# Baran-phys/IEA-GAN

Hardware: AMD Instinct MI355X
Metric: events/sec (40x250x768) per G+D train step (higher is better)
Workload: dtype bf16; 1 GPU; BASELINE configs[1]: 1 event (40x1x256x768) per GPU per step, hinge loss only, RRM on, DiffAugment on, ortho reg + Adam + EMA in the timed region, fp32 master weights, 4 synthetic events in rotation; parallelism=dp1, hip_graph=True

## Files before the change

iea-gan_amd/_hip.py:

```python
from __future__ import annotations

import ctypes as C
import os

import torch

_HERE = os.path.dirname(os.path.abspath(__file__))
LIB_PATH = os.path.join(_HERE, "libieagan_hip.so")
CONV_FP8_NOSCALE = 8
CONV_FP8 = 4
CONV_NO_LDS_WEIGHTS = 2
CONV_FORCE_GATHER = 1
B1_OCC2, B1_OCC3, B1_TP32 = 1, 2, 4
BWD_NO_REDUCE = 16
PXD_BINS = 251
PXD_CLUSTER_COLUMNS = {"size_spectrum": (0, 64), "charge_spectrum": (64, 256), "seed_spectrum": (320, 256), "size_u_spectrum": (576, 32),
                       "size_v_spectrum": (608, 32)}
PXD_CLUSTER_BINS = 640
PROLOGUE_BWD_SLOTS = 64
AUG_SLOTS = 128
BNB_REPL = 8
STAT_REPL = 32
SN_FIELDS = 16

vp, fp, lp, ip = C.c_void_p, C.c_void_p, C.c_void_p, C.c_void_p


class SrcDesc(C.Structure):
    _fields_ = [("x", vp), ("Cx", C.c_int), ("Hs", C.c_int), ("Ws", C.c_int), ("rs", C.c_int),
                ("scale", vp), ("shift", vp), ("aff_nstride", C.c_int), ("relu", C.c_int)]


class ConvDesc(C.Structure):
    _fields_ = [("N", C.c_int), ("H", C.c_int), ("W", C.c_int), ("Cin", C.c_int), ("Cout", C.c_int),
                ("taps", C.c_int), ("Kpad", C.c_int), ("src", SrcDesc), ("w", vp), ("bias", vp),
                ("ra", vp), ("Cra", C.c_int), ("Ca", C.c_int), ("ra_rs", C.c_int), ("ra_scale", C.c_float), ("rb", vp),
                ("Crb", C.c_int), ("mask", vp), ("out", vp), ("stats", vp), ("n_per_event", C.c_int), ("flags", C.c_int),
                ("bnb_scale", vp), ("bnb_shift", vp), ("bnb_nstride", C.c_int), ("bnb_relu", C.c_int), ("stats_slots", C.c_int)]


class WgradDesc(C.Structure):
# ... 21 lines not shown

class DStemDesc(C.Structure):
    _fields_ = [("img", vp), ("N", C.c_int), ("H", C.c_int), ("W", C.c_int), ("w_in", vp), ("b_in", vp), ("w1", vp), ("b1", vp), ("wsc", vp),
                ("bsc", vp), ("h1", vp), ("p0", vp), ("sc", vp), ("dh1", vp), ("dp0", vp), ("w1_bwd", vp), ("dw_in", vp), ("db_in", vp),
                ("dw1", vp), ("db1", vp)]


class ProfRec(C.Structure):
    _fields_ = [("name", C.c_char * 96), ("launches", C.c_long), ("ms", C.c_double),
                ("flops", C.c_double), ("bytes", C.c_double), ("bytes_min", C.c_double)]


ABI_VERSION = 12
i, f, l = C.c_int, C.c_float, C.c_long
_SIGS = {
    "ieagan_abi_version": [],
    "ieagan_prof_enable": [i],
    "ieagan_prof_reset": [],
    "ieagan_prof_collect": [C.POINTER(ProfRec), i],
    "ieagan_conv_forward": [C.POINTER(ConvDesc), vp],
    "ieagan_conv_wgrad": [C.POINTER(WgradDesc), i, vp],
    "ieagan_conv_wgrad_workspace": [C.POINTER(WgradDesc), i],
    "ieagan_conv1x1_bwd": [C.POINTER(Conv1x1BwdDesc), vp],
    "ieagan_conv1x1_bwd_workspace": [C.POINTER(Conv1x1BwdDesc)],
    "ieagan_conv1x1_bwd_supported": [i, i, i, i],
    "ieagan_conv3x3_bwd": [C.POINTER(Conv3x3BwdDesc), vp],
    "ieagan_conv3x3_bwd_workspace": [C.POINTER(Conv3x3BwdDesc)],
    "ieagan_conv3x3_bwd_supported": [i, i, i, i, i, i, i],
    "ieagan_conv3x3_bwd_slots": [C.POINTER(Conv3x3BwdDesc)],
    "ieagan_conv1x1_bwd_slots": [C.POINTER(Conv1x1BwdDesc)],
    "ieagan_wgrad_reduce": [vp, vp, i, i, i, i, vp],
    "ieagan_wgrad_reduce_batched": [C.POINTER(ReduceItem), i, vp],
    "ieagan_conv_stats_slots": [C.POINTER(ConvDesc)],
    "ieagan_d_stem_fwd": [C.POINTER(DStemDesc), vp],
    "ieagan_d_stem_bwd": [C.POINTER(DStemDesc), vp],
    "ieagan_effgrad": [vp, vp, vp, vp, vp, l, i, i, vp],
    "ieagan_prologue_bwd": [vp, vp, i, vp, vp, i, i, i, vp, vp, vp, i, i, i, i, vp, i, i, i, i, vp],
    "ieagan_bn_finalize_fwd": [vp, f, vp, vp, i, i, f, f, i, vp, vp, vp, vp, vp, i, i, i, i, vp, vp],
    "ieagan_bn_finalize_bwd": [vp, vp, vp, i, i, vp, f, i, vp, vp, i, vp, i, i, i, i, vp, vp],
    "ieagan_bn_finalize_fwd_scratch": [i, i, i],
    "ieagan_bn_finalize_bwd_scratch": [i, i, i, i],
    "ieagan_res_bwd": [vp, i, vp, i, i, i, i, i, i, vp],
    "ieagan_nchw_to_nhwc": [vp, vp, vp, i, i, i, i, vp],
    "ieagan_nhwc_to_nchw": [vp, vp, i, i, i, vp],
    "ieagan_channel_stats": [vp, vp, l, i, vp],
    "ieagan_conv_1toC": [vp, vp, vp, vp, vp, i, i, i, i, i, vp],
    "ieagan_conv_1toC_bnb": [vp, vp, vp, vp, vp, vp, i, i, vp, vp, vp, i, i, i, i, i, i, vp],
    "ieagan_conv_1toC_bnb_slots": [i, i, i, i],
    "ieagan_conv_Cto1": [vp, vp, vp, i, i, vp, vp, vp, i, i, i, i, i, i, vp],
    "ieagan_wgrad_c1": [vp, vp, vp, vp, vp, i, i, vp, i, i, i, i, i, vp],
    "ieagan_sn_backward_batched": [vp, vp, i, vp, vp, vp, vp, vp],
    "ieagan_sn_forward": [vp, vp, i, vp, i, vp, vp, vp, vp, f, i, vp],
    "ieagan_sn_backward": [vp, vp, i, i, i, i, i, i, vp, vp, vp, i, vp, vp, i, vp],
    "ieagan_sn_backward_stack": [vp, vp, vp, vp, i, vp, vp, vp, vp, i, vp],
    "ieagan_nl_attention_fwd": [vp, vp, vp, vp, vp, i, i, i, i, i, vp],
    "ieagan_nl_attention_bwd": [vp, vp, vp, vp, vp, vp, vp, vp, vp, vp, i, i, i, i, i, vp],
    "ieagan_rrm_attention_fwd": [vp, vp, vp, i, i, i, i, vp],
    "ieagan_rrm_attention_bwd": [vp, vp, vp, vp, i, i, i, i, vp],
    "ieagan_slin_fwd": [vp, vp, vp, vp, vp, vp, vp, vp, vp, i, i, i, i, f, vp],
    "ieagan_slin_bwd": [vp, vp, vp, vp, vp, vp, vp, vp, vp, vp, i, i, i, i, vp],
    "ieagan_ln_fwd": [vp, vp, vp, vp, vp, vp, i, i, f, i, vp],
    "ieagan_ln_bwd": [vp, vp, vp, vp, vp, vp, vp, vp, vp, i, i, vp],
    "ieagan_embed_norm_fwd": [vp, vp, vp, vp, i, i, vp],
    "ieagan_embed_norm_bwd": [vp, vp, vp, vp, vp, i, i, vp],
    "ieagan_loss_block": [vp, vp, vp, vp, vp, C.POINTER(C.c_float), f, vp, vp, vp, vp, vp, i, i, vp],
    "ieagan_loss_block_events": [vp, vp, vp, vp, vp, C.POINTER(C.c_float), f, vp, vp, vp, vp, vp, i, i, i, vp],
# ... 82 lines not shown
```

iea-gan_amd/csrc/api.hip:

```cpp
#include <stdarg.h>
#include <stdio.h>
#include <string.h>

#include <map>
#include <mutex>
#include <string>
#include <vector>

#include "common.h"
#include "conv_args.h"

static thread_local char g_err[512] = "";

void ieagan_set_error(const char* fmt, ...) {
    va_list ap;
    va_start(ap, fmt);
    vsnprintf(g_err, sizeof(g_err), fmt, ap);
    va_end(ap);
}

extern "C" const char* ieagan_last_error(void) { return g_err; }
extern "C" int ieagan_abi_version(void) { return IEAGAN_ABI_VERSION; }

struct ProfEvt {
// ... 66 lines not shown
            strncpy(r.name, e.name.c_str(), sizeof(r.name) - 1);
        }
        r.launches += 1;
        r.ms += ms;
        r.flops += e.flops;
        r.bytes += e.bytes;
        r.bytes_min += e.bytes_min;
    }
    prof_clear_locked();
    int n = 0;
    for (auto& kv : agg) {
        if (n >= cap) break;
        out[n++] = kv.second;
    }
    return n;
}

extern "C" int ieagan_conv_forward(const ieagan_conv_desc* d, void* stream) {
    CHECK_ARG(d != nullptr && d->src.x != nullptr && d->w != nullptr && d->out != nullptr, "conv_forward: null pointer");
    return conv_gather_launch(*d, (hipStream_t)stream);
}

extern "C" int ieagan_conv_stats_slots(const ieagan_conv_desc* d) {
    CHECK_ARG(d != nullptr, "conv_stats_slots: null pointer");
    g_plan.on = true;
    g_plan.slots = -1;
    const int rc = conv_gather_launch(*d, nullptr);
    g_plan.on = false;
    if (rc < 0) return rc;
    CHECK_ARG(g_plan.slots > 0, "conv_stats_slots: the dispatch reached no launch site");
    return g_plan.slots;
}

extern "C" int ieagan_conv_wgrad(const ieagan_wgrad_desc* d, int use_tr_read, void* stream) {
    CHECK_ARG(d != nullptr && d->src.x != nullptr && d->g != nullptr && d->dw != nullptr, "conv_wgrad: null pointer");
    return conv_wgrad_launch(*d, (hipStream_t)stream, use_tr_read);
}

__global__ void selftest_tr_kernel(const bf16* __restrict__ in, bf16* __restrict__ out) {
    __shared__ __attribute__((aligned(16))) bf16 lds[64 * 16];
    const int l = threadIdx.x;
    for (int i = l; i < 64 * 16; i += 64) lds[i] = in[i];
    __syncthreads();
    const int lr = l & 15, lg = l >> 4;
    const int q = lr >> 2, p = lr & 3;
    const bf16* p0 = lds + (8 * lg + q) * 16 + 4 * p;
    const bf16* p1 = p0 + 4 * 16;
    const bf16x4 lo = __builtin_amdgcn_ds_read_tr16_b64_v4bf16((bf16x4 __attribute__((address_space(3)))*)p0);
    const bf16x4 hi = __builtin_amdgcn_ds_read_tr16_b64_v4bf16((bf16x4 __attribute__((address_space(3)))*)p1);
#pragma unroll
    for (int j = 0; j < 4; ++j) {
        out[l * 8 + j] = lo[j];
        out[l * 8 + 4 + j] = hi[j];
    }
}

extern "C" int ieagan_selftest_tr_read(const void* in, void* out, void* stream) {
    hipLaunchKernelGGL(selftest_tr_kernel, dim3(1), dim3(64), 0, (hipStream_t)stream, (const bf16*)in, (bf16*)out);
    CHECK_LAUNCH("selftest_tr_read");
    return 0;
}
```

iea-gan_amd/csrc/conv1x1_tile.hip:

```cpp
#include "common.h"
#include "conv_args.h"
#include "conv_common.h"

namespace {

template <int KC>
__device__ __forceinline__ int tkey(int r) { return KC == 128 ? (r & 15) : KC == 64 ? ((r >> 1) & 7) : ((r >> 2) & 3); }
template <int KC>
__device__ __forceinline__ int toff(int r, int c) { return r * KC + ((c ^ tkey<KC>(r)) << 3); }

template <bool AFF, bool RELU>
__device__ __forceinline__ void pro8(float (&v)[8], const bf16x8& raw, const SrcDesc& s, int n, int c, const float* aff) {
#pragma unroll
    for (int i = 0; i < 8; ++i) v[i] = bf2f(raw[i]);
    xform8<AFF, RELU>(v, s, n, c, aff);
}

}

template <bool AFF, bool RELU, int RS, int NT, int KC, bool BNB>
__global__ __launch_bounds__(256, 3) void conv1x1_tile_kernel(ConvArgs a) {
    constexpr int CPR = KC / 8;
    constexpr int EROWS = 16;
    constexpr int ABYTES = 128 * KC * 2, BBYTES = NT * 16 * KC * 2;
    constexpr int EPIB = 4 * EROWS * EpiLds<NT>::LDW * 4;
    constexpr int ASZ = ABYTES > EPIB ? ABYTES : EPIB;
    static_assert(EPIB >= 4 * STATS_SX_FLOATS * 4, "epilogue buffer doubles as the statistics scratch");
    __shared__ __attribute__((aligned(16))) char smem[ASZ + BBYTES];
    __shared__ float red[4 * NT * 16 * 2];
    __shared__ __attribute__((aligned(32))) float aff_s[AFF ? 2 * AFF_MAXC : 8];
    bf16* atile = (bf16*)smem;
    bf16* btile = (bf16*)(smem + ASZ);
    float* epi = (float*)smem;
    const int lane = threadIdx.x & 63, wave = threadIdx.x >> 6;
    const int lr = lane & 15, lg = lane >> 4;
    const int H = a.H, W = a.W, HW = H * W;
    const long M = (long)a.N * HW;
    const int gy = a.Cout / (NT * 16);
    int vid = blockIdx.x;
    {
        const int tot = gridDim.x, q = tot / 8, r = tot % 8, xcd = vid % 8;
        vid = (xcd < r ? xcd * (q + 1) : r * (q + 1) + (xcd - r) * q) + vid / 8;
    }
    const int bx = vid / gy;
    const long m_blk = (long)bx * 128;
    const long m_base = m_blk + wave * 32;
    const int n_base = (vid % gy) * NT * 16;
    const int n_img = (int)(m_blk / HW);
    if (AFF) stage_aff(aff_s, a.src, n_img, a.Cin);
    const float* affp = AFF ? aff_s : nullptr;
    const bf16* xsrc = (const bf16*)a.src.x;

    f32x4 acc[2][NT];
#pragma unroll
// ... 80 lines not shown
                    for (int q = 0; q < 4; ++q) {
                        float v[8];
                        pro8<AFF, RELU>(v, raw[jj][q], a.src, n, min(ch, a.Cin - 8), affp);
#pragma unroll
                        for (int i = 0; i < 8; ++i) s8[i] += v[i];
                    }
                    bf16x8 o;
#pragma unroll
                    for (int i = 0; i < 8; ++i) o[i] = f2bf(0.25f * s8[i]);
                    if (m_blk + p >= M || ch >= a.Cin) o = zero8();
                    *(bf16x8*)(atile + toff<KC>(p, c)) = o;
                }
            }
        }
        __syncthreads();
#pragma unroll
        for (int ks = 0; ks < KC / 32; ++ks) {
            bf16x8 af[2], bf[NT];
#pragma unroll
            for (int mt = 0; mt < 2; ++mt) af[mt] = *(const bf16x8*)(atile + toff<KC>(wave * 32 + mt * 16 + lr, ks * 4 + lg));
#pragma unroll
            for (int nt = 0; nt < NT; ++nt) bf[nt] = *(const bf16x8*)(btile + toff<KC>(nt * 16 + lr, ks * 4 + lg));
#pragma unroll
            for (int mt = 0; mt < 2; ++mt)
#pragma unroll
                for (int nt = 0; nt < NT; ++nt) acc[mt][nt] = __builtin_amdgcn_mfma_f32_16x16x32_bf16(af[mt], bf[nt], acc[mt][nt], 0, 0, 0);
        }
    }
    __syncthreads();

    float s1[8], s2[8];
#pragma unroll
    for (int i = 0; i < 8; ++i) s1[i] = s2[i] = 0.f;
    const bool need_hw = (a.ra != nullptr && a.ra_rs != 0) || (BNB && a.bnb_scale != nullptr);
    auto pix = [&](int row, long& m, int& n, int& h, int& w) -> bool {
        m = m_base + row;
        n = h = w = 0;
        if (m >= M) return false;
        if (need_hw) {
            n = (int)(m / HW);
            const int rem = (int)(m - (long)n * HW);
            h = rem / W;
            w = rem - h * W;
        }
        return true;
    };
#pragma unroll
    for (int half = 0; half < 2; ++half) {
        auto pixh = [&](int row, long& m, int& n, int& h, int& w) -> bool { return pix(row + 16 * half, m, n, h, w); };
        const f32x4(&sub)[1][NT] = *reinterpret_cast<const f32x4(*)[1][NT]>(&acc[half]);
        conv_epilogue<BNB, NT, 1, (RS != 2)>(a, sub, epi + wave * EROWS * EpiLds<NT>::LDW, n_base, pixh, s1, s2);
    }
    if (a.stats != nullptr) {
        __syncthreads();
        const int event = (a.n_per_event > 0) ? (int)(m_blk / ((long)a.n_per_event * HW)) : 0;
        stats_flush<NT>(a, s1, s2, n_base, red, epi, bx, event);
    }
}

template <bool AFF, bool RELU, int RS, bool BNB>
static int tile_dispatch(const ConvArgs& a, hipStream_t st) {
    const long M = (long)a.N * a.H * a.W;
    const unsigned gx = (unsigned)((M + 127) / 128);
    const int n_events_t = (a.stats != nullptr && a.n_per_event > 0) ? a.N / a.n_per_event : 1;
#define TL(NTV, KCV)                                                                                                                    \
    {                                                                                                                                   \
        CONV_PLAN_POINT((int)(gx / n_events_t), 1)                                                                                      \
        hipLaunchKernelGGL((conv1x1_tile_kernel<AFF, RELU, RS, NTV, KCV, BNB>), dim3(gx * (a.Cout / (NTV * 16))), dim3(256), 0, st, a);     \
        return 1;                                                                                                                       \
    }
#define BY_KC(NTV)                      \
    if (a.Cin <= 32) TL(NTV, 32)        \
    else if (a.Cin == 64) TL(NTV, 64)   \
    else TL(NTV, 128)
    if (a.Cout % 64 == 0) { BY_KC(4) }
    else { BY_KC(2) }
#undef BY_KC
#undef TL
    return 0;
}

int conv1x1_tile_launch(const ConvArgs& a, hipStream_t st) {
    if (a.taps != 1 || (a.src.rs != 0 && a.src.rs != 2) || a.Cout % 32 != 0 || a.Cin % 8 != 0) return 0;
    if (!(a.Cin <= 32 || a.Cin == 64 || a.Cin % 128 == 0) || a.Kpad != ((a.Cin + 31) / 32) * 32) return 0;
    const long HW = (long)a.H * a.W, M = (long)a.N * HW;
    if (M < (a.src.rs == 2 ? 1024 : 4096)) return 0;
    if (M < 16384 && a.Cin > 256) return 0;
    const bool aff = a.src.scale != nullptr, relu = a.src.relu != 0;
    if (aff && (HW % 128 != 0 || a.Cin > AFF_MAXC)) return 0;
    if (a.bnb_scale != nullptr) {
        if (aff || relu || a.src.rs != 0) return 0;
        return tile_dispatch<false, false, 0, true>(a, st);
    }
    if (a.src.rs == 0) {
        if (aff && relu) return tile_dispatch<true, true, 0, false>(a, st);
        if (aff) return tile_dispatch<true, false, 0, false>(a, st);
        if (relu) return tile_dispatch<false, true, 0, false>(a, st);
        return tile_dispatch<false, false, 0, false>(a, st);
    }
    if (aff && relu) return tile_dispatch<true, true, 2, false>(a, st);
    if (aff) return tile_dispatch<true, false, 2, false>(a, st);
    if (relu) return tile_dispatch<false, true, 2, false>(a, st);
    return tile_dispatch<false, false, 2, false>(a, st);
}
```

iea-gan_amd/csrc/conv_common.h:

```cpp
#pragma once
#include "common.h"
#include "conv_args.h"

#define AFF_MAXC 512
__device__ __forceinline__ void stage_aff(float* aff, const SrcDesc& s, int n, int Cin) {
    for (int i = threadIdx.x; i < Cin; i += 256) {
        aff[i] = s.scale[(long)n * s.aff_nstride + i];
        aff[AFF_MAXC + i] = s.shift[(long)n * s.aff_nstride + i];
    }
}

template <bool AFF, bool RELU>
__device__ __forceinline__ void xform8(float (&v)[8], const SrcDesc& s, int n, int c, const float* aff = nullptr) {
    if (AFF) {
        f32x8 sc, sh;
        if (aff != nullptr) {
            typedef const __attribute__((address_space(3))) f32x8* lds_f32x8;
            sc = *(lds_f32x8)(aff + c);
            sh = *(lds_f32x8)(aff + AFF_MAXC + c);
        } else {
            sc = *(const f32x8*)(s.scale + (long)n * s.aff_nstride + c);
            sh = *(const f32x8*)(s.shift + (long)n * s.aff_nstride + c);
        }
#pragma unroll
// ... 169 lines not shown
                int n, h, w;
                long mm;
                pix(row, mm, n, h, w);
                const bf16* p = (const bf16*)a.ra + (((long)n * (2 * H) + 2 * h) * (2 * W) + 2 * w) * a.Cra + co0;
                const long rs_ = (long)2 * W * a.Cra;
                const bf16x8 t0 = *(const bf16x8*)p, t1 = *(const bf16x8*)(p + a.Cra), t2 = *(const bf16x8*)(p + rs_),
                             t3 = *(const bf16x8*)(p + rs_ + a.Cra);
#pragma unroll
                for (int i = 0; i < 8; ++i) rv[i] = 0.25f * (bf2f(t0[i]) + bf2f(t1[i]) + bf2f(t2[i]) + bf2f(t3[i]));
            }
#pragma unroll
            for (int i = 0; i < 8; ++i) v[i] += a.ra_scale * rv[i];
        } else if (rb_here) {
            const bf16x8 t = EARLY ? rs_r[it] : *(const bf16x8*)((const bf16*)a.rb + m * a.Crb + (co0 - a.Ca));
#pragma unroll
            for (int i = 0; i < 8; ++i) v[i] += bf2f(t[i]);
        }
        bf16x8 o;
#pragma unroll
        for (int i = 0; i < 8; ++i) {
            o[i] = f2bf(v[i]);
            if (!bnb) {
                s1[i] += v[i];
                s2[i] += v[i] * v[i];
            }
        }
        *(bf16x8*)((bf16*)a.out + m * a.Cout + co0) = o;
    }
    __builtin_amdgcn_fence(__ATOMIC_SEQ_CST, "wavefront");
    __builtin_amdgcn_wave_barrier();
}


template <bool AFF, bool RELU, int RS>
__device__ __forceinline__ bf16x8 gather8(const SrcDesc& s, int H, int W, int n, int hh, int ww, int c, bool ok,
                                          const float* aff = nullptr) {
    ok = ok && (hh >= 0) && (hh < H) && (ww >= 0) && (ww < W);
    if (!ok) return zero8();
    if (RS == 2) {
        float acc[8];
#pragma unroll
        for (int i = 0; i < 8; ++i) acc[i] = 0.f;
#pragma unroll
        for (int q = 0; q < 4; ++q) {
            const bf16x8 raw = *(const bf16x8*)((const bf16*)s.x + (((long)n * s.Hs + 2 * hh + (q >> 1)) * s.Ws + 2 * ww + (q & 1)) * s.Cx + c);
            float v[8];
#pragma unroll
            for (int i = 0; i < 8; ++i) v[i] = bf2f(raw[i]);
            xform8<AFF, RELU>(v, s, n, c, aff);
#pragma unroll
            for (int i = 0; i < 8; ++i) acc[i] += v[i];
        }
        bf16x8 o;
#pragma unroll
        for (int i = 0; i < 8; ++i) o[i] = f2bf(0.25f * acc[i]);
        return o;
    }
    const int sh_ = (RS == 1) ? (hh >> 1) : hh, sw_ = (RS == 1) ? (ww >> 1) : ww;
    const bf16x8 raw = *(const bf16x8*)((const bf16*)s.x + (((long)n * s.Hs + sh_) * s.Ws + sw_) * s.Cx + c);
    if (!AFF && !RELU) return raw;
    if (!AFF && RELU) return relu8(raw);
    float v[8];
#pragma unroll
    for (int i = 0; i < 8; ++i) v[i] = bf2f(raw[i]);
    xform8<AFF, RELU>(v, s, n, c, aff);
    bf16x8 o;
// ... 6 lines not shown
```

iea-gan_amd/csrc/conv_igemm.hip:

```cpp
#include "common.h"
#include "conv_args.h"
#include "conv_common.h"
#include <stdio.h>

template <int TAPS, bool AFF, bool RELU, int RS, int NT, bool LAFF, bool BNB = false>
__global__ __launch_bounds__(256, 4) void conv_gather_kernel(ConvArgs a) {
    constexpr int EROWS = (NT >= 2) ? 16 : 32;
    __shared__ __attribute__((aligned(16))) float epi[4 * EROWS * EpiLds<NT>::LDW];
    __shared__ float red[4 * NT * 16 * 2];
    __shared__ __attribute__((aligned(32))) float aff_s[LAFF ? 2 * AFF_MAXC : 8];
    const int lane = threadIdx.x & 63, wave = threadIdx.x >> 6;
    const int lr = lane & 15, lg = lane >> 4;
    const int H = a.H, W = a.W, HW = H * W;
    const long M = (long)a.N * HW;
    const bool sk = NT == 1 && (a.flags & CONV_INTERNAL_SPLITK) != 0;
    const int ppb = sk ? 32 : 128;
    const long m_base = sk ? (long)blockIdx.x * 32 : ((long)blockIdx.x * 4 + wave) * 32;
    const int n_base = blockIdx.y * NT * 16;

    int pn[2], ph[2], pw[2];
    bool pv[2];
#pragma unroll
    for (int mt = 0; mt < 2; ++mt) {
        const long m = m_base + mt * 16 + lr;
// ... 428 lines not shown
    const bool small = ntiles * ((a.Cout + 63) / 64) < 512;
    const bool kp_ok = a.Kpad == ((9 * a.Cin + 31) / 32) * 32;
    if (!kp_ok) {
        if (a.Cout % 64 == 0 && !small) HALO_LAUNCH(4, 0, 0)
        else if (a.Cout % 32 == 0 && !(small && ntiles * (a.Cout / 32) < 512)) HALO_LAUNCH(2, 0, 0)
        else HALO_LAUNCH(1, 0, 0)
    }
    else if (a.Cin == 16 && a.Cout == 16) HALO_LAUNCH(1, 3, 16)
    else if (a.Cin == 32 && a.Cout == 32) HALO_LAUNCH(2, 6, 32)
    else if (a.Cin == 64 && a.Cout == 64 && ntiles >= 1024) HALO_LAUNCH(4, 11, 64)
    else if (a.Cin == 64 && a.Cout % 64 == 0 && !small) HALO_LAUNCH(4, 0, 64)
    else if (a.Cin == 128 && a.Cout % 64 == 0 && !small) HALO_LAUNCH(4, 0, 128)
    else if (a.Cin == 128 && a.Cout % 32 == 0 && !(small && ntiles * (a.Cout / 32) < 512)) HALO_LAUNCH(2, 0, 128)
    else if (a.Cin == 64 && a.Cout % 32 == 0 && !(small && ntiles * (a.Cout / 32) < 512)) HALO_LAUNCH(2, 0, 64)
    else if (a.Cout % 64 == 0 && !small) HALO_LAUNCH(4, 0, 0)
    else if (a.Cout % 32 == 0 && !(small && ntiles * (a.Cout / 32) < 512)) HALO_LAUNCH(2, 0, 0)
    else HALO_LAUNCH(1, 0, 0)
#undef HALO_LAUNCH
    return 0;
}

template <int RS>
static int launch_halo_pro(const ConvArgs& a, hipStream_t st) {
    const bool aff = a.src.scale != nullptr, relu = a.src.relu != 0;
    if (aff && relu) return launch_halo_nt<true, true, RS>(a, st);
    if (aff) return launch_halo_nt<true, false, RS>(a, st);
    if (relu) return launch_halo_nt<false, true, RS>(a, st);
    if (RS == 0 && a.bnb_scale != nullptr) return launch_halo_nt<false, false, (RS == 0 ? 0 : RS), (RS == 0)>(a, st);
    return launch_halo_nt<false, false, RS>(a, st);
}

int conv_gather_launch(const ConvArgs& a, hipStream_t st) {
    CHECK_ARG(a.taps == 1 || a.taps == 9, "conv: taps must be 1 or 9 (got %d)", a.taps);
    CHECK_ARG((a.flags & ~(IEAGAN_CONV_FORCE_GATHER | IEAGAN_CONV_NO_LDS_WEIGHTS | IEAGAN_CONV_FP8 | IEAGAN_CONV_FP8_NOSCALE)) == 0, "conv: unknown flag bits 0x%x", a.flags);
    CHECK_ARG(a.Cin % 8 == 0 && a.Cout % 8 == 0, "conv: Cin/Cout must be multiples of 8 (%d,%d)", a.Cin, a.Cout);
    CHECK_ARG(a.Kpad % 32 == 0 && a.Kpad >= a.taps * a.Cin, "conv: bad Kpad %d", a.Kpad);
    CHECK_ARG(a.src.rs >= 0 && a.src.rs <= 2, "conv: bad resample mode %d", a.src.rs);
    CHECK_ARG(a.src.Cx % 8 == 0, "conv: source channel stride must be a multiple of 8");
    CHECK_ARG((a.src.scale == nullptr) == (a.src.shift == nullptr), "conv: scale/shift must come together");
    if (a.src.rs == 1) CHECK_ARG(a.H == 2 * a.src.Hs && a.W == 2 * a.src.Ws, "conv: upsample geometry mismatch");
    if (a.src.rs == 2) CHECK_ARG(2 * a.H == a.src.Hs && 2 * a.W == a.src.Ws, "conv: pool geometry mismatch");
    if (a.src.rs == 0) CHECK_ARG(a.H == a.src.Hs && a.W == a.src.Ws, "conv: geometry mismatch");
    if (a.ra) CHECK_ARG(a.Ca <= a.Cout && a.Ca <= a.Cra && a.Ca % 8 == 0 && a.Cra % 8 == 0, "conv: residual channel slice out of range");
    if (a.ra && a.ra_rs == 1) CHECK_ARG(a.H % 2 == 0 && a.W % 2 == 0, "conv: upsampled residual needs even H, W");
    if (a.rb) CHECK_ARG(a.Crb % 8 == 0 && a.Crb >= a.Cout - a.Ca, "conv: bad residual-B channel count");
    CHECK_ARG(a.n_per_event >= 0 && (a.n_per_event == 0 || a.N % a.n_per_event == 0), "conv: N=%d is not a whole number of events of %d images", a.N, a.n_per_event);
    if (a.bnb_scale != nullptr)
        CHECK_ARG(a.src.scale == nullptr && a.src.relu == 0 && a.src.rs == 0 && a.bnb_shift != nullptr && a.mask != nullptr && a.stats != nullptr && a.n_per_event == 1 && a.bias == nullptr && a.Cout % 8 == 0 &&
                  (a.bnb_nstride == 0 || a.bnb_nstride >= a.Cout), "conv: BatchNorm-backward epilogue needs a plain prologue, shift, x (mask), per-image accumulators (n_per_event = 1), no bias");
    if (a.stats != nullptr && a.n_per_event > 0 && a.n_per_event < a.N)
        CHECK_ARG(((long)a.n_per_event * a.H * a.W) % 128 == 0, "conv: per-event statistics need n_per_event*H*W %% 128 == 0 (%d*%d*%d)", a.n_per_event, a.H, a.W);
    const double flops = 2.0 * a.N * a.H * a.W * (double)a.Cout * a.taps * a.Cin;
    double bytes = 2.0 * a.N * ((double)a.src.Hs * a.src.Ws * a.Cin + (double)a.H * a.W * a.Cout);
    const double bytes_min = bytes;
    if (a.mask) bytes += 2.0 * a.N * (double)a.H * a.W * a.Cout;
    if (a.ra) bytes += 2.0 * a.N * (double)a.H * a.W * a.Ca * (a.ra_rs == 1 ? 0.25 : (a.ra_rs == 2 ? 4.0 : 1.0));
    if (a.rb) bytes += 2.0 * a.N * (double)a.H * a.W * (a.Cout - a.Ca);
    const bool halo = a.taps == 9 && a.src.rs != 2 && a.W >= 16 && a.H >= 4 && a.Cin % 16 == 0 && !(a.flags & IEAGAN_CONV_FORCE_GATHER) &&
                      (size_t)(HT_H + 2) * (HT_W + 2) * (a.Cin * 2 + 16) <= 150 * 1024 && a.Cin <= AFF_MAXC;
    char tag[64] = "";
    if (prof_tags_on())
        snprintf(tag, sizeof(tag), "ci%d co%d %dx%d rs%d a%d r%d res%d%s", a.Cin, a.Cout, a.H, a.W, a.src.rs, a.src.scale != nullptr,
                 a.src.relu, a.ra ? a.ra_rs + 1 : 0, a.mask ? " mask" : "");
    ProfScope prof(a.taps == 9 ? (halo ? "conv3x3_halo" : "conv3x3_gather") : "conv1x1_gather", flops, bytes, st, tag, bytes_min);
    int rc;
    if (halo) {
        rc = (a.flags & IEAGAN_CONV_NO_LDS_WEIGHTS) ? 0 : conv3x3_lds_launch(a, st);
        if (rc < 0) return rc;
        if (rc == 0 && !(a.flags & IEAGAN_CONV_NO_LDS_WEIGHTS)) rc = conv3x3_ws_launch(a, st);
        if (rc < 0) return rc;
        if (rc == 0) rc = (a.src.rs == 0) ? launch_halo_pro<0>(a, st) : launch_halo_pro<1>(a, st);
        else rc = 0;
    } else if (a.taps == 9) {
        if (a.src.rs == 0) rc = launch_gather_pro<9, 0>(a, st);
        else if (a.src.rs == 1) rc = launch_gather_pro<9, 1>(a, st);
        else { ieagan_set_error("conv: 3x3 with pooled source is not instantiated"); return IEAGAN_EINVAL; }
    } else {
        if (a.src.rs == 0) {
            if (!(a.flags & IEAGAN_CONV_FORCE_GATHER) && conv1x1_stream_launch(a, st)) rc = 0;
            else if (!(a.flags & IEAGAN_CONV_FORCE_GATHER) && conv1x1_tile_launch(a, st)) rc = 0;
            else rc = launch_gather_pro<1, 0>(a, st);
        }
        else if (a.src.rs == 2) {
            if (!(a.flags & IEAGAN_CONV_FORCE_GATHER) && conv1x1_tile_launch(a, st)) rc = 0;
            else rc = launch_gather_pro<1, 2>(a, st);
        }
        else { ieagan_set_error("conv: 1x1 with upsampled source is not instantiated"); return IEAGAN_EINVAL; }
    }
    if (conv_plan_ctx().on) return rc;
    CHECK_LAUNCH("conv_forward");
    return rc;
}
```

iea-gan_amd/ops.py:

```python
from __future__ import annotations

import math
import types
from typing import Optional

import torch

import _hip as H
from _hip import STAT_REPL

BF16 = torch.bfloat16


def _kpad(k: int) -> int:
    return (k + 31) // 32 * 32


class _ZeroPool:
    CHUNK = 8 << 20

    def __init__(self):
        self.buf, self.pos = {}, {}

    def take(self, n: int, device) -> torch.Tensor:
# ... 16 lines not shown


def reset_zero_pool():
    _ZEROS.reset()


def zeros(shape, device) -> torch.Tensor:
    n = 1
    for d in (shape if isinstance(shape, (tuple, list, torch.Size)) else (shape,)):
        n *= int(d)
    return _ZEROS.take(n, device).view(shape)


def new_stats(C: int, device, events: int = 1, slots: int = STAT_REPL) -> torch.Tensor:
    return zeros((events, slots, 2, C), device)


DIRECT_GRADS = False


class direct_grads:
    def __enter__(self):
        global DIRECT_GRADS
        self.prev, DIRECT_GRADS = DIRECT_GRADS, True

    def __exit__(self, *a):
        global DIRECT_GRADS
        DIRECT_GRADS = self.prev


class ExecOptions:
    FIELDS = dict(wgrad_side_stream=True, two_stage_wgrad=True, fuse_bn_backward=True, fuse_shortcut_grad=True,
                  fuse_1x1_backward=True, fuse_1x1_min_pixels=1 << 16, fuse_3x3_backward=True, fuse_3x3_min_pixels=1 << 16,
                  fuse_d_stem=True)
    __slots__ = tuple(FIELDS)

    def __init__(self, like=None, **kw):
        src = like if like is not None else globals().get("DEFAULTS")
        for k, v in self.FIELDS.items():
            setattr(self, k, getattr(src, k) if src is not None else v)
        self.update(**kw)

    def update(self, **kw):
        for k, v in kw.items():
            if k not in self.FIELDS:
                raise KeyError(f"unknown execution option {k!r} (have: {sorted(self.FIELDS)})")
            setattr(self, k, v)
        return self

    def as_dict(self):
        return {k: getattr(self, k) for k in self.FIELDS}


DEFAULTS = ExecOptions()


def opts_of(rec) -> "ExecOptions":
    ps = getattr(rec, "pass_", None)
    return ps.bank.opts if ps is not None else DEFAULTS


def opts_of_net(net) -> "ExecOptions":
    return (net if isinstance(net, SNBank) else net._prepare()["bank"]).opts


def set_options(net, **kw) -> "ExecOptions":
    bank = net if isinstance(net, SNBank) else net._prepare()["bank"]
# ... 390 lines not shown
        rows = 1 if events == 1 else n_images
        shape = (C,) if rows == 1 else (rows, C)
        scale = torch.empty(shape, dtype=torch.float32, device=dev)
        shift = torch.empty(shape, dtype=torch.float32, device=dev)
        mr = torch.empty(events, 2, C, dtype=torch.float32, device=dev)
        repl = int(stats.shape[1]) if stats is not None else 0
        H.call("ieagan_bn_finalize_fwd", H.ptr(stats), float(count), gain.data_ptr(), bias.data_ptr(), 0, 0, float(eps),
               float(momentum), int(training), run_mean.data_ptr(), run_var.data_ptr(), scale.data_ptr(),
               shift.data_ptr(), mr.data_ptr(), rows, C, events, repl,
               H.ptr(_fin_scratch("fwd", C, events, repl, device=dev) if training else None), H.stream())
        ctx.count, ctx.training, ctx.has_stats, ctx.events, ctx.rows, ctx.repl = count, training, stats is not None, events, rows, repl
        ctx.save_for_backward(gain, mr)
        return scale, shift

    @staticmethod
    def backward(ctx, dscale, dshift):
        gain, mr = ctx.saved_tensors
        C = gain.numel()
        dev = gain.device
        E, rows = ctx.events, ctx.rows
        dgain, dbias = torch.empty_like(gain), torch.empty_like(gain)
        dstat = torch.empty(E, 2, C, dtype=torch.float32, device=dev)
        shape = (C,) if rows == 1 else (rows, C)
        dscale = dscale.contiguous() if dscale is not None else torch.zeros(shape, device=dev)
        dshift = dshift.contiguous() if dshift is not None else torch.zeros(shape, device=dev)
        H.call("ieagan_bn_finalize_bwd", dscale.data_ptr(), dshift.data_ptr(), gain.data_ptr(), 0, 0, mr.data_ptr(),
               float(ctx.count), int(ctx.training), dgain.data_ptr(), dbias.data_ptr(), 0, dstat.data_ptr(), rows, C, E, 0,
               None, H.stream())
        dstats = dstat.unsqueeze(1).expand(E, ctx.repl, 2, C) if (ctx.has_stats and ctx.training) else None
        return dstats, dgain, dbias, None, None, None, None, None, None, None, None


def _conv_launch(x, Cx, Hs, Ws, rs, scale, shift, nstride, relu, N, Hc, Wc, Cin, Cout, taps, kpad, w, bias,
                 ra, Cra, Ca, ra_rs, rb, Crb, mask, out, stats, ra_scale=1.0, npe=0, flags=0, bnb=None):
    bs, bt, bn, br = (H.ptr(bnb[0]), H.ptr(bnb[1]), int(bnb[2]), int(bool(bnb[3]))) if bnb is not None else (None, None, 0, 0)
    alloc = stats is True
    d = H.ConvDesc(N, Hc, Wc, Cin, Cout, taps, kpad, H.src_desc(x, Cx, Hs, Ws, rs, scale, shift, nstride, relu),
                   H.ptr(w), H.ptr(bias), H.ptr(ra), Cra, Ca, ra_rs, float(ra_scale), H.ptr(rb), Crb, H.ptr(mask),
                   H.ptr(out), 16 if alloc else H.ptr(stats), int(npe), int(flags), bs, bt, bn, br,
                   0 if (alloc or stats is None) else int(stats.shape[1]))
    if alloc:
        slots = H.lib().ieagan_conv_stats_slots(d)
        if slots <= 0:
            raise RuntimeError(f"ieagan_conv_stats_slots failed ({slots}): {H.lib().ieagan_last_error().decode()}")
        stats = zeros((N // npe if npe else 1, slots, 2, Cout), out.device)
        d.stats, d.stats_slots = stats.data_ptr(), slots
    H.call("ieagan_conv_forward", d, H.stream())
    return stats


_WGRAD_STREAMS = {}


def wgrad_stream(device) -> "torch.cuda.Stream":
    key = (torch.device(device).index or 0, torch.cuda.current_stream(device).cuda_stream)
    if key not in _WGRAD_STREAMS:
        _WGRAD_STREAMS[key] = torch.cuda.Stream(device=device)
    return _WGRAD_STREAMS[key]


def release_device_caches():
    _ZEROS.reset()
    _WGRAD_STREAMS.clear()
    _PLACEHOLDERS.clear()


class BNLink:
    __slots__ = ("acc",)

    def __init__(self):
        self.acc = None

class ResLink:
# ... 81 lines not shown
            b.res_out.deposit(gl, gl.stride()[2] if not gl.is_contiguous() else b.Cout, b.Ca, b.ra_rs)
        elif b.ra_rs == 0:
            if b.Ca == b.Cout and rshape[-1] == b.Cout:
                d_ra = gl
            else:
                d_ra = torch.zeros(rshape, dtype=BF16, device=b.dev)
                d_ra[..., :b.Ca] = gl[..., :b.Ca]
        else:
            d_ra = torch.empty(rshape, dtype=BF16, device=b.dev)
            H.call("ieagan_res_bwd", gl.contiguous().data_ptr(), b.Cout, d_ra.data_ptr(), rshape[-1], b.Ca, b.ra_rs, b.N, rshape[1], rshape[2],
                   H.stream())
    if b.has_rb and b.need[6]:
        d_rb = gl[..., b.Ca:]
    return d_ra, d_rb


def _fused_buffers(d, kernel, N, Cin, has_aff, dev):
    acc = ws = None
    if has_aff:
        d.bn_slots = getattr(H.lib(), f"ieagan_{kernel}_slots")(d)
        if d.bn_slots <= 0:
            raise RuntimeError(f"ieagan_{kernel}_slots failed: {H.lib().ieagan_last_error().decode()}")
        acc = zeros((N, d.bn_slots, 2, Cin), dev)
        d.bn_acc = acc.data_ptr()
    ws_n = getattr(H.lib(), f"ieagan_{kernel}_workspace")(d)
    if ws_n < 0:
        raise RuntimeError(f"ieagan_{kernel}_workspace failed: {H.lib().ieagan_last_error().decode()}")
    if ws_n > 0:
        ws = torch.empty(ws_n, dtype=torch.float32, device=dev)
        d.partials = ws.data_ptr()
    return acc, ws


def _dgrad(b, g, Cg, out, *, link=None, link_rs=0, link_scale=1.0, mask=None, stats=None, bnb=None, flags=0, npe=0):
    lg, lC, lCa = link if link is not None else (None, 0, 0)
    return _conv_launch(g, Cg, b.Hc, b.Wc, 0, None, None, 0, False, b.N, b.Hc, b.Wc, b.Cout, b.Cin, b.taps, b.rec.kpad2, b.rec.w_bwd, None,
                        lg, lC, lCa, link_rs, None, 0, mask, out, stats, ra_scale=link_scale, npe=npe, flags=flags, bnb=bnb)


def _conv_grads(dx=None, dW=None, dbias=None, dscale=None, dshift=None, d_ra=None, d_rb=None):
    return (dx, dW, dbias, dscale, dshift, d_ra, d_rb) + (None,) * 11


def _fused_bwd_launch(name, d, rec, ws, dwp, Cout, K):
    pass_ = getattr(rec, "pass_", None)
    batched = ws is not None and getattr(rec, "deferred", False) and pass_ is not None and pass_.arena is not None
    if batched:
        d.flags |= H.BWD_NO_REDUCE
    H.call(name, d, H.stream())
    if batched:
        pass_.reduces.append((ws, dwp, ws.numel() // (Cout * rec.kpad), Cout, rec.kpad, K))


def _fused_1x1_eligible(b, dout, dstats):
    rec, o, rs, relu, has_aff, res_out, res_in, need = b.rec, b.opts, b.rs, b.relu, b.has_aff, b.res_out, b.res_in, b.need
    if not o.fuse_1x1_backward:
        return False
    if b.taps != 1 or rs not in (0, 2) or not need[0] or not need[1] or b.Wc % 32 != 0 or b.N * b.Hc * b.Wc < o.fuse_1x1_min_pixels:
        return False
    if not H.lib().ieagan_conv1x1_bwd_supported(rec.cin, rec.out, rs, int(has_aff)):
        return False
    if isinstance(res_in, SumLink) or (has_aff and (rs != 0 or b.events > 1 and b.nstride == 0)):
        return False
    if res_in is not None and res_in.ready:
        if rs == 2 and not (res_out is None and not relu and not has_aff):
            return False
        if rs == 0 and res_in.mode not in (0, 1, 2):
            return False
    elif rs == 2 and res_out is None and not relu and res_in is not None:
        return False
# ... 82 lines not shown
    if dstats is not None:
        geff = torch.empty_like(g)
        if b.has_bias:
            colsum = sn_scratch(rec, "b", (STAT_REPL, Cout), dev) if (need[1] and need[2]) else zeros((STAT_REPL, Cout), dev)
        H.call("ieagan_effgrad", g.data_ptr(), b.out.data_ptr(), dstats[:, 0].contiguous().data_ptr(), geff.data_ptr(),
               H.ptr(colsum), P, Cout, b.events, H.stream())
        g = geff
    elif b.has_bias and need[2]:
        colsum = sn_scratch(rec, "b", (STAT_REPL, Cout), dev) if need[1] else zeros((STAT_REPL, Cout), dev)
        if need[1]:
            colsum_in_wgrad = True
        else:
            H.call("ieagan_effgrad", g.data_ptr(), None, None, None, colsum.data_ptr(), P, Cout, 1, H.stream())
    return g, Cg, colsum, colsum_in_wgrad


def _prologue_bwd(b, da, link, rmode):
    if rmode == 2:
        raise RuntimeError("pooled shortcut gradient cannot be added by prologue_bwd")
    dx = torch.empty(b.N, b.Hs, b.Ws, b.Cin, dtype=BF16, device=b.dev)
    acc = zeros((b.N, H.PROLOGUE_BWD_SLOTS, 2, b.Cin), b.dev) if b.has_aff else None
    H.call("ieagan_prologue_bwd", da.data_ptr(), b.x.data_ptr(), b.Cx, H.ptr(b.scale), H.ptr(b.shift), b.nstride, int(b.relu),
           b.rs, dx.data_ptr(), H.ptr(acc), None, b.N, b.Hs, b.Ws, b.Cin, H.ptr(link[0]), link[1], link[2], rmode,
           H.PROLOGUE_BWD_SLOTS if b.has_aff else 0, H.stream())
    return (dx,) + (_bn_param_grads(b.scale, acc, b.nstride) if b.has_aff else (None, None))


def _data_gradient(b, g, Cg):
    x, scale, rs, relu, has_aff, res_in = b.x, b.scale, b.rs, b.relu, b.has_aff, b.res_in
    N, Hs, Ws, Cin, dev = b.N, b.Hs, b.Ws, b.Cin, b.dev
    dx = dscale = dshift = None
    if not (b.need[0] or (has_aff and (b.need[3] or b.need[4]))):
        return dx, dscale, dshift
    da = torch.empty(N, b.Hc, b.Wc, Cin, dtype=BF16, device=dev)
    fuse_mask = relu and not has_aff and rs == 0
    plain = not relu and not has_aff
    lg = lC = lCa = lmode = None
    fan_in = res_in if isinstance(res_in, SumLink) else None
    if res_in is not None and not res_in.ready:
        res_in = None
    if res_in is not None:
        lg, lC, lCa, lmode = res_in.take()
    link = (lg, lC or 0, lCa or 0)
    bn_link = getattr(scale, "_bn_link", None) if has_aff else None
    if (b.opts.fuse_bn_backward and has_aff and rs == 0 and bn_link is not None and (Hs * Ws) % 128 == 0 and Cin % 8 == 0
            and (res_in is None or lmode in (0, 1))):
        dx = torch.empty(N, Hs, Ws, Cin, dtype=BF16, device=dev)
        up = res_in is not None and lmode == 1
        acc = _dgrad(b, g, Cg, dx, link=link, link_rs=2 if up else 0, link_scale=4.0 if up else 1.0, mask=x, stats=True,
                     bnb=(scale, b.shift, b.nstride, relu), flags=b.flags, npe=1)
        dscale, dshift = _bn_param_grads(scale, acc, b.nstride)
    elif res_in is not None and (fuse_mask or (plain and rs == 0)):
        _dgrad(b, g, Cg, da, link=link, link_rs=1 if lmode == 2 else 0, link_scale=0.25 if lmode == 2 else 1.0,
               mask=x if fuse_mask else None, flags=b.flags)
        dx = da
    elif res_in is not None and plain and rs == 2 and b.res_out is None:
        _dgrad(b, g, Cg, da, link=link)
        res_in.deposit(da, Cin, Cin, 2)
    else:
        _dgrad(b, g, Cg, da, mask=x if fuse_mask else None, flags=b.flags)
        if (fuse_mask or (plain and rs == 0)) and res_in is None:
            dx = da
        else:
            dx, dscale, dshift = _prologue_bwd(b, da, link, lmode if res_in is not None else 0)
    if fan_in is not None:
        if not (plain and rs == 0 and dx is da):
# ... 645 lines not shown
```

include/ieagan_hip.h:

```cpp
#ifndef IEAGAN_HIP_H
#define IEAGAN_HIP_H
#include <stddef.h>
#ifdef __cplusplus
extern "C" {
#endif

const char* ieagan_last_error(void);
#define IEAGAN_ABI_VERSION 12
int ieagan_abi_version(void);

int ieagan_prof_enable(int on);
int ieagan_prof_reset(void);
typedef struct { char name[96]; long launches; double ms; double flops; double bytes; double bytes_min; } ieagan_prof_rec;
int ieagan_prof_collect(ieagan_prof_rec* out, int cap);

typedef struct {
    const void* x;
    int Cx, Hs, Ws;
    int rs;
    const float* scale;
    const float* shift;
    int aff_nstride;
    int relu;
} ieagan_src_desc;

typedef struct {
    int N, H, W;
    int Cin, Cout, taps;
    int Kpad;
    ieagan_src_desc src;
    const void* w;
    const float* bias;
    const void* ra;
    int Cra, Ca, ra_rs;
    float ra_scale;
    const void* rb;
    int Crb;
    const void* mask;
    void* out;
    float* stats;
    int n_per_event;
    int flags;
    const float* bnb_scale;
    const float* bnb_shift;
    int bnb_nstride;
    int bnb_relu;
    int stats_slots;
} ieagan_conv_desc;
#define IEAGAN_CONV_FORCE_GATHER 1
#define IEAGAN_CONV_FP8 4
#define IEAGAN_CONV_FP8_NOSCALE 8
#define IEAGAN_CONV_NO_LDS_WEIGHTS 2
int ieagan_conv_forward(const ieagan_conv_desc* d, void* stream);
int ieagan_conv_stats_slots(const ieagan_conv_desc* d);

typedef struct {
    int N, H, W;
    int Cin, Cout, taps, Kpad;
    ieagan_src_desc src;
    const void* g;
    int Cg;
    float* dw;
    int tiles_per_block;
    int pad_rows;
    float* partials;
    float* colsum;
} ieagan_wgrad_desc;
int ieagan_conv_wgrad(const ieagan_wgrad_desc* d, int use_tr_read, void* stream);
long ieagan_conv_wgrad_workspace(const ieagan_wgrad_desc* d, int use_tr_read);

typedef struct {
    int N, H, W;
    int Cin, Cout, Kpad, Kpad2;
    ieagan_src_desc src;
    const void* g;
    int Cg;
    const void* y;
    const float* dstat;
    int n_per_event;
    void* geff_out;
    const void* w_bwd;
    const void* lg;
    int lC, lCa, lmode;
    void* dx;
    int out_mode;
    float* bn_acc;
// ... 183 lines not shown
```

Baseline: 30.56 events/s.

## Fuse avg-pool backward and ReLU mask into 1x1 dgrad tile epilogue

Adds a pooled-source dgrad path for 1x1 convs whose input was ReLU'd and 2x2 average-pooled. The tile kernel's epilogue now scatters the quarter-scaled gradient to the four full-resolution pixels, masked by the sign of x. This replaces writing an intermediate pooled-resolution gradient and then running a separate prologue-backward pass. A plan-mode query checks shape support first and falls back to the old path otherwise. The cost is an extra kernel instantiation and scattered 4x stores from the epilogue, and the gradient is rounded to bf16 before the 0.25 scale.

```diff
diff --git a/iea-gan_amd/_hip.py b/iea-gan_amd/_hip.py
--- a/iea-gan_amd/_hip.py
+++ b/iea-gan_amd/_hip.py
@@ -7,6 +7,7 @@
 
 _HERE = os.path.dirname(os.path.abspath(__file__))
 LIB_PATH = os.path.join(_HERE, "libieagan_hip.so")
+CONV_POOL_BWD = 16
 CONV_FP8_NOSCALE = 8
 CONV_FP8 = 4
 CONV_NO_LDS_WEIGHTS = 2
@@ -94,6 +95,7 @@
     "ieagan_wgrad_reduce": [vp, vp, i, i, i, i, vp],
     "ieagan_wgrad_reduce_batched": [C.POINTER(ReduceItem), i, vp],
     "ieagan_conv_stats_slots": [C.POINTER(ConvDesc)],
+    "ieagan_conv_pool_bwd_supported": [C.POINTER(ConvDesc)],
     "ieagan_d_stem_fwd": [C.POINTER(DStemDesc), vp],
     "ieagan_d_stem_bwd": [C.POINTER(DStemDesc), vp],
     "ieagan_effgrad": [vp, vp, vp, vp, vp, l, i, i, vp],
diff --git a/iea-gan_amd/csrc/api.hip b/iea-gan_amd/csrc/api.hip
--- a/iea-gan_amd/csrc/api.hip
+++ b/iea-gan_amd/csrc/api.hip
@@ -122,6 +122,15 @@
     return g_plan.slots;
 }
 
+extern "C" int ieagan_conv_pool_bwd_supported(const ieagan_conv_desc* d) {
+    CHECK_ARG(d != nullptr, "conv_pool_bwd_supported: null pointer");
+    g_plan.on = true;
+    g_plan.slots = -1;
+    const int rc = conv_gather_launch(*d, nullptr);
+    g_plan.on = false;
+    return rc == 0 ? 1 : 0;
+}
+
 extern "C" int ieagan_conv_wgrad(const ieagan_wgrad_desc* d, int use_tr_read, void* stream) {
     CHECK_ARG(d != nullptr && d->src.x != nullptr && d->g != nullptr && d->dw != nullptr, "conv_wgrad: null pointer");
     return conv_wgrad_launch(*d, (hipStream_t)stream, use_tr_read);
diff --git a/iea-gan_amd/csrc/conv1x1_tile.hip b/iea-gan_amd/csrc/conv1x1_tile.hip
--- a/iea-gan_amd/csrc/conv1x1_tile.hip
+++ b/iea-gan_amd/csrc/conv1x1_tile.hip
@@ -18,8 +18,8 @@
 
 }
 
-template <bool AFF, bool RELU, int RS, int NT, int KC, bool BNB>
-__global__ __launch_bounds__(256, 3) void conv1x1_tile_kernel(ConvArgs a) {
+template <bool AFF, bool RELU, int RS, int NT, int KC, bool BNB, bool PBWD>
+__device__ __forceinline__ void conv1x1_tile_body(const ConvArgs a) {
     constexpr int CPR = KC / 8;
     constexpr int EROWS = 16;
     constexpr int ABYTES = 128 * KC * 2, BBYTES = NT * 16 * KC * 2;
@@ -166,7 +166,7 @@
     float s1[8], s2[8];
 #pragma unroll
     for (int i = 0; i < 8; ++i) s1[i] = s2[i] = 0.f;
-    const bool need_hw = (a.ra != nullptr && a.ra_rs != 0) || (BNB && a.bnb_scale != nullptr);
+    const bool need_hw = PBWD || (a.ra != nullptr && a.ra_rs != 0) || (BNB && a.bnb_scale != nullptr);
     auto pix = [&](int row, long& m, int& n, int& h, int& w) -> bool {
         m = m_base + row;
         n = h = w = 0;
@@ -183,13 +183,24 @@
     for (int half = 0; half < 2; ++half) {
         auto pixh = [&](int row, long& m, int& n, int& h, int& w) -> bool { return pix(row + 16 * half, m, n, h, w); };
         const f32x4(&sub)[1][NT] = *reinterpret_cast<const f32x4(*)[1][NT]>(&acc[half]);
-        conv_epilogue<BNB, NT, 1, (RS != 2)>(a, sub, epi + wave * EROWS * EpiLds<NT>::LDW, n_base, pixh, s1, s2);
-    }
-    if (a.stats != nullptr) {
+        if (PBWD) conv_epilogue_pool_bwd<NT>(a, sub, epi + wave * EROWS * EpiLds<NT>::LDW, n_base, pixh);
+        else conv_epilogue<BNB, NT, 1, (RS != 2)>(a, sub, epi + wave * EROWS * EpiLds<NT>::LDW, n_base, pixh, s1, s2);
+    }
+    if (!PBWD && a.stats != nullptr) {
         __syncthreads();
         const int event = (a.n_per_event > 0) ? (int)(m_blk / ((long)a.n_per_event * HW)) : 0;
         stats_flush<NT>(a, s1, s2, n_base, red, epi, bx, event);
     }
+}
+
+template <bool AFF, bool RELU, int RS, int NT, int KC, bool BNB>
+__global__ __launch_bounds__(256, 3) void conv1x1_tile_kernel(ConvArgs a) {
+    conv1x1_tile_body<AFF, RELU, RS, NT, KC, BNB, false>(a);
+}
+
+template <int NT>
+__global__ __launch_bounds__(256, 3) void conv1x1_tile_poolbwd_kernel(ConvArgs a) {
+    conv1x1_tile_body<false, false, 0, NT, 128, false, true>(a);
 }
 
 template <bool AFF, bool RELU, int RS, bool BNB>
@@ -214,7 +225,19 @@
     return 0;
 }
 
+static int tile_poolbwd_launch(const ConvArgs& a, hipStream_t st) {
+    if (a.Cin % 128 != 0 || a.Kpad != a.Cin || a.Cout % 32 != 0) return 0;
+    const long M = (long)a.N * a.H * a.W;
+    if (M < 4096 || (M < 16384 && a.Cin > 256)) return 0;
+    const unsigned gx = (unsigned)((M + 127) / 128);
+    CONV_PLAN_POINT((int)gx, 1)
+    if (a.Cout % 64 == 0) hipLaunchKernelGGL((conv1x1_tile_poolbwd_kernel<4>), dim3(gx * (a.Cout / 64)), dim3(256), 0, st, a);
+    else hipLaunchKernelGGL((conv1x1_tile_poolbwd_kernel<2>), dim3(gx * (a.Cout / 32)), dim3(256), 0, st, a);
+    return 1;
+}
+
 int conv1x1_tile_launch(const ConvArgs& a, hipStream_t st) {
+    if (a.flags & IEAGAN_CONV_POOL_BWD) return tile_poolbwd_launch(a, st);
     if (a.taps != 1 || (a.src.rs != 0 && a.src.rs != 2) || a.Cout % 32 != 0 || a.Cin % 8 != 0) return 0;
     if (!(a.Cin <= 32 || a.Cin == 64 || a.Cin % 128 == 0) || a.Kpad != ((a.Cin + 31) / 32) * 32) return 0;
     const long HW = (long)a.H * a.W, M = (long)a.N * HW;
diff --git a/iea-gan_amd/csrc/conv_common.h b/iea-gan_amd/csrc/conv_common.h
--- a/iea-gan_amd/csrc/conv_common.h
+++ b/iea-gan_amd/csrc/conv_common.h
@@ -225,6 +225,65 @@
 }
 
 
+template <int NT, typename PixFn>
+__device__ __forceinline__ void conv_epilogue_pool_bwd(const ConvArgs& a, const f32x4 (&acc)[1][NT], float* wlds, int n_base, PixFn pix) {
+    constexpr int LDW = EpiLds<NT>::LDW;
+    constexpr int CPP = NT * 2;
+    constexpr int EIT = (16 * CPP) / 64;
+    static_assert((16 * CPP) % 64 == 0, "epilogue rows x chunks must fill whole waves");
+    const int lane = threadIdx.x & 63;
+    const int lr = lane & 15, lg = lane >> 4;
+#pragma unroll
+    for (int nt = 0; nt < NT; ++nt)
+#pragma unroll
+        for (int r = 0; r < 4; ++r) wlds[(lg * 4 + r) * LDW + nt * 16 + lr] = acc[0][nt][r];
+    __builtin_amdgcn_fence(__ATOMIC_SEQ_CST, "wavefront");
+    __builtin_amdgcn_wave_barrier();
+    const int cc = lane % CPP;
+    const int co0 = n_base + cc * 8;
+    const long ps = a.Cout, rs_ = (long)2 * a.W * a.Cout;
+    bf16x8 xk[EIT][4];
+    long o_r[EIT];
+    bool ok_r[EIT];
+#pragma unroll
+    for (int it = 0; it < EIT; ++it) {
+        const int row = (it * 64 + lane) / CPP;
+        long m;
+        int n, h, w;
+        ok_r[it] = pix(row, m, n, h, w) && co0 < a.Cout;
+        o_r[it] = (((long)n * (2 * a.H) + 2 * h) * (2 * a.W) + 2 * w) * a.Cout + co0;
+#pragma unroll
+        for (int q = 0; q < 4; ++q) xk[it][q] = zero8();
+        if (!ok_r[it]) continue;
+        const bf16* p = (const bf16*)a.mask + o_r[it];
+        xk[it][0] = *(const bf16x8*)p;
+        xk[it][1] = *(const bf16x8*)(p + ps);
+        xk[it][2] = *(const bf16x8*)(p + rs_);
+        xk[it][3] = *(const bf16x8*)(p + rs_ + ps);
+    }
+#pragma unroll
+    for (int it = 0; it < EIT; ++it) {
+        const int row = (it * 64 + lane) / CPP;
+        const f32x4 lo = *(const f32x4*)(wlds + row * LDW + cc * 8);
+        const f32x4 hi = *(const f32x4*)(wlds + row * LDW + cc * 8 + 4);
+        if (!ok_r[it]) continue;
+        float d[8];
+#pragma unroll
+        for (int i = 0; i < 8; ++i) d[i] = 0.25f * bf2f(f2bf(i < 4 ? lo[i & 3] : hi[i & 3]));
+        bf16* p = (bf16*)a.out + o_r[it];
+#pragma unroll
+        for (int q = 0; q < 4; ++q) {
+            bf16x8 o;
+#pragma unroll
+            for (int i = 0; i < 8; ++i) o[i] = f2bf(bf2f(xk[it][q][i]) > 0.f ? d[i] : 0.f);
+            *(bf16x8*)(p + (q >> 1) * rs_ + (q & 1) * ps) = o;
+        }
+    }
+    __builtin_amdgcn_fence(__ATOMIC_SEQ_CST, "wavefront");
+    __builtin_amdgcn_wave_barrier();
+}
+
+
 template <bool AFF, bool RELU, int RS>
 __device__ __forceinline__ bf16x8 gather8(const SrcDesc& s, int H, int W, int n, int hh, int ww, int c, bool ok,
                                           const float* aff = nullptr) {
diff --git a/iea-gan_amd/csrc/conv_igemm.hip b/iea-gan_amd/csrc/conv_igemm.hip
--- a/iea-gan_amd/csrc/conv_igemm.hip
+++ b/iea-gan_amd/csrc/conv_igemm.hip
@@ -484,7 +484,7 @@
 
 int conv_gather_launch(const ConvArgs& a, hipStream_t st) {
     CHECK_ARG(a.taps == 1 || a.taps == 9, "conv: taps must be 1 or 9 (got %d)", a.taps);
-    CHECK_ARG((a.flags & ~(IEAGAN_CONV_FORCE_GATHER | IEAGAN_CONV_NO_LDS_WEIGHTS | IEAGAN_CONV_FP8 | IEAGAN_CONV_FP8_NOSCALE)) == 0, "conv: unknown flag bits 0x%x", a.flags);
+    CHECK_ARG((a.flags & ~(IEAGAN_CONV_FORCE_GATHER | IEAGAN_CONV_NO_LDS_WEIGHTS | IEAGAN_CONV_FP8 | IEAGAN_CONV_FP8_NOSCALE | IEAGAN_CONV_POOL_BWD)) == 0, "conv: unknown flag bits 0x%x", a.flags);
     CHECK_ARG(a.Cin % 8 == 0 && a.Cout % 8 == 0, "conv: Cin/Cout must be multiples of 8 (%d,%d)", a.Cin, a.Cout);
     CHECK_ARG(a.Kpad % 32 == 0 && a.Kpad >= a.taps * a.Cin, "conv: bad Kpad %d", a.Kpad);
     CHECK_ARG(a.src.rs >= 0 && a.src.rs <= 2, "conv: bad resample mode %d", a.src.rs);
@@ -502,10 +502,16 @@
                   (a.bnb_nstride == 0 || a.bnb_nstride >= a.Cout), "conv: BatchNorm-backward epilogue needs a plain prologue, shift, x (mask), per-image accumulators (n_per_event = 1), no bias");
     if (a.stats != nullptr && a.n_per_event > 0 && a.n_per_event < a.N)
         CHECK_ARG(((long)a.n_per_event * a.H * a.W) % 128 == 0, "conv: per-event statistics need n_per_event*H*W %% 128 == 0 (%d*%d*%d)", a.n_per_event, a.H, a.W);
+    const bool pool_bwd = (a.flags & IEAGAN_CONV_POOL_BWD) != 0;
+    if (pool_bwd)
+        CHECK_ARG(a.taps == 1 && a.src.rs == 0 && a.src.scale == nullptr && a.src.relu == 0 && a.mask != nullptr && a.bias == nullptr && a.ra == nullptr &&
+                  a.rb == nullptr && a.stats == nullptr && a.bnb_scale == nullptr && !(a.flags & IEAGAN_CONV_FORCE_GATHER),
+                  "conv: the pooled-source dgrad epilogue needs a plain 1x1 launch with x as the mask and no other epilogue operand");
     const double flops = 2.0 * a.N * a.H * a.W * (double)a.Cout * a.taps * a.Cin;
     double bytes = 2.0 * a.N * ((double)a.src.Hs * a.src.Ws * a.Cin + (double)a.H * a.W * a.Cout);
     const double bytes_min = bytes;
-    if (a.mask) bytes += 2.0 * a.N * (double)a.H * a.W * a.Cout;
+    if (a.mask) bytes += 2.0 * a.N * (double)a.H * a.W * a.Cout * (pool_bwd ? 4.0 : 1.0);
+    if (pool_bwd) bytes += 2.0 * a.N * (double)a.H * a.W * a.Cout * 3.0;
     if (a.ra) bytes += 2.0 * a.N * (double)a.H * a.W * a.Ca * (a.ra_rs == 1 ? 0.25 : (a.ra_rs == 2 ? 4.0 : 1.0));
     if (a.rb) bytes += 2.0 * a.N * (double)a.H * a.W * (a.Cout - a.Ca);
     const bool halo = a.taps == 9 && a.src.rs != 2 && a.W >= 16 && a.H >= 4 && a.Cin % 16 == 0 && !(a.flags & IEAGAN_CONV_FORCE_GATHER) &&
@@ -516,7 +522,10 @@
                  a.src.relu, a.ra ? a.ra_rs + 1 : 0, a.mask ? " mask" : "");
     ProfScope prof(a.taps == 9 ? (halo ? "conv3x3_halo" : "conv3x3_gather") : "conv1x1_gather", flops, bytes, st, tag, bytes_min);
     int rc;
-    if (halo) {
+    if (pool_bwd) {
+        if (conv1x1_tile_launch(a, st)) rc = 0;
+        else { ieagan_set_error("conv: the pooled-source dgrad epilogue is not instantiated for this shape (ieagan_conv_pool_bwd_supported)"); return IEAGAN_EINVAL; }
+    } else if (halo) {
         rc = (a.flags & IEAGAN_CONV_NO_LDS_WEIGHTS) ? 0 : conv3x3_lds_launch(a, st);
         if (rc < 0) return rc;
         if (rc == 0 && !(a.flags & IEAGAN_CONV_NO_LDS_WEIGHTS)) rc = conv3x3_ws_launch(a, st);
diff --git a/iea-gan_amd/ops.py b/iea-gan_amd/ops.py
--- a/iea-gan_amd/ops.py
+++ b/iea-gan_amd/ops.py
@@ -72,7 +72,7 @@
 class ExecOptions:
     FIELDS = dict(wgrad_side_stream=True, two_stage_wgrad=True, fuse_bn_backward=True, fuse_shortcut_grad=True,
                   fuse_1x1_backward=True, fuse_1x1_min_pixels=1 << 16, fuse_3x3_backward=True, fuse_3x3_min_pixels=1 << 16,
-                  fuse_d_stem=True)
+                  fuse_d_stem=True, fuse_pool_dgrad=True)
     __slots__ = tuple(FIELDS)
 
     def __init__(self, like=None, **kw):
@@ -529,13 +529,15 @@
 
 
 def _conv_launch(x, Cx, Hs, Ws, rs, scale, shift, nstride, relu, N, Hc, Wc, Cin, Cout, taps, kpad, w, bias,
-                 ra, Cra, Ca, ra_rs, rb, Crb, mask, out, stats, ra_scale=1.0, npe=0, flags=0, bnb=None):
+                 ra, Cra, Ca, ra_rs, rb, Crb, mask, out, stats, ra_scale=1.0, npe=0, flags=0, bnb=None, query=None):
     bs, bt, bn, br = (H.ptr(bnb[0]), H.ptr(bnb[1]), int(bnb[2]), int(bool(bnb[3]))) if bnb is not None else (None, None, 0, 0)
     alloc = stats is True
     d = H.ConvDesc(N, Hc, Wc, Cin, Cout, taps, kpad, H.src_desc(x, Cx, Hs, Ws, rs, scale, shift, nstride, relu),
                    H.ptr(w), H.ptr(bias), H.ptr(ra), Cra, Ca, ra_rs, float(ra_scale), H.ptr(rb), Crb, H.ptr(mask),
                    H.ptr(out), 16 if alloc else H.ptr(stats), int(npe), int(flags), bs, bt, bn, br,
                    0 if (alloc or stats is None) else int(stats.shape[1]))
+    if query is not None:
+        return getattr(H.lib(), query)(d)
     if alloc:
         slots = H.lib().ieagan_conv_stats_slots(d)
         if slots <= 0:
@@ -683,10 +685,10 @@
     return acc, ws
 
 
-def _dgrad(b, g, Cg, out, *, link=None, link_rs=0, link_scale=1.0, mask=None, stats=None, bnb=None, flags=0, npe=0):
+def _dgrad(b, g, Cg, out, *, link=None, link_rs=0, link_scale=1.0, mask=None, stats=None, bnb=None, flags=0, npe=0, query=None):
     lg, lC, lCa = link if link is not None else (None, 0, 0)
     return _conv_launch(g, Cg, b.Hc, b.Wc, 0, None, None, 0, False, b.N, b.Hc, b.Wc, b.Cout, b.Cin, b.taps, b.rec.kpad2, b.rec.w_bwd, None,
-                        lg, lC, lCa, link_rs, None, 0, mask, out, stats, ra_scale=link_scale, npe=npe, flags=flags, bnb=bnb)
+                        lg, lC, lCa, link_rs, None, 0, mask, out, stats, ra_scale=link_scale, npe=npe, flags=flags, bnb=bnb, query=query)
 
 
 def _conv_grads(dx=None, dW=None, dbias=None, dscale=None, dshift=None, d_ra=None, d_rb=None):
@@ -835,6 +837,13 @@
     dx = dscale = dshift = None
     if not (b.need[0] or (has_aff and (b.need[3] or b.need[4]))):
         return dx, dscale, dshift
+    if (b.opts.fuse_pool_dgrad and b.taps == 1 and rs == 2 and relu and not has_aff and res_in is None and b.Cx == Cin
+            and Hs == 2 * b.Hc and Ws == 2 * b.Wc):
+        dx = torch.empty(N, Hs, Ws, Cin, dtype=BF16, device=dev)
+        if _dgrad(b, g, Cg, dx, mask=x, flags=H.CONV_POOL_BWD, query="ieagan_conv_pool_bwd_supported") == 1:
+            _dgrad(b, g, Cg, dx, mask=x, flags=H.CONV_POOL_BWD)
+            return dx, dscale, dshift
+        dx = None
     da = torch.empty(N, b.Hc, b.Wc, Cin, dtype=BF16, device=dev)
     fuse_mask = relu and not has_aff and rs == 0
     plain = not relu and not has_aff
diff --git a/include/ieagan_hip.h b/include/ieagan_hip.h
--- a/include/ieagan_hip.h
+++ b/include/ieagan_hip.h
@@ -51,7 +51,9 @@
 #define IEAGAN_CONV_FP8 4
 #define IEAGAN_CONV_FP8_NOSCALE 8
 #define IEAGAN_CONV_NO_LDS_WEIGHTS 2
+#define IEAGAN_CONV_POOL_BWD 16
 int ieagan_conv_forward(const ieagan_conv_desc* d, void* stream);
+int ieagan_conv_pool_bwd_supported(const ieagan_conv_desc* d);
 int ieagan_conv_stats_slots(const ieagan_conv_desc* d);
 
 typedef struct {
```

New measurement: 30.69 events/s (median of 6 runs). About the same (+0.4%).
